# rbrito/deprecated-lame-mirror

Measured on AMD Instinct MI355X. Metric: encoded audio seconds/sec (x real-time) at 44.1kHz stereo CBR128, higher is better.
Workload: dtype f32

## Files before the change

### deprecated-lame-mirror_amd/csrc/lh_dev_common.h

```cpp
#ifndef LH_DEV_COMMON_H
#define LH_DEV_COMMON_H

#include <stdint.h>
#include "lamehip_types.h"
#include "lh_device.h"
#include "lh_wave.h"
#include "lh_dev_math.h"

#define LH_NT 128
#ifdef LH_LSF
#define LH_NGR 1
#define LH_IS_LSF 1
#define LH_RATE8K(c) ((c).rate8k)
#else
#define LH_NGR 2
#define LH_IS_LSF 0
#define LH_RATE8K(c) 0
#endif
#define LH_BLOCK LH_NT
#define LH_SQRT2 1.41421356237309504880

#ifdef LH_EMU
#define LH_SYNC_WG() do { __syncthreads(); } while (0)
#define LH_SYNC_WG_LDS() do { __syncthreads(); } while (0)
// ... 284 lines not shown

struct LhVbrSave {
    uint8_t sfwork[LH_SFBMAX + 1];
    uint8_t sfmin[LH_SFBMAX + 1];
    int     mingain_l, mingain_s[3];
    int     global_gain, mnc, max_bits, use_bits;
    int     ath_over, nonzero, pad[2];
    int     table_select[3], region0_count, region1_count, pad2[3];
};

#if !(defined(LH_PROF) && !defined(LH_EMU))
#define LH_VBR_OLD 1
#endif

struct LhVbrOldSave {
    LhQR    R;
    LhGrR   g;
    uint8_t sf[LH_SFBMAX + 1];
    float   xmin[LH_SFBMAX + 1];
    int     used_bits, fin_bits;
    int     ath_over, pad;
};

struct LhQuantLds {
    LhChanLds ch[2];
};
static_assert(__builtin_offsetof(LhTables, pow43) % 128 == 0 && __builtin_offsetof(LhTables, vqthr) % 128 == 0
              && __builtin_offsetof(LhTables, vq3) % 128 == 0,
              "the gathered tables start on cache lines (hipMalloc aligns the struct itself)");
static_assert(sizeof(LhChanLds) % 16 == 0, "both channels' float2/float4 accesses need 16-byte alignment");
static_assert(__builtin_offsetof(LhPsyLds, mid.small) >= __builtin_offsetof(LhChanLds, ix[1]) + sizeof(((LhChanLds *) 0)->ix[1])
              && __builtin_offsetof(LhPsyLds, mid.lng) + sizeof(LhMidLong) <= sizeof(LhChanLds) + __builtin_offsetof(LhChanLds, ix[1])
              && __builtin_offsetof(LhPsyLds, mid.small) % 16 == 0,
              "the staged mid record lies between the two channels' second images (log table / VBR step tables)");

#define LH_VBR_IPOW20 ((float *) lh_lds.u.quant.ch[0].ix[1])
#define LH_VBR_POW20  ((float *) lh_lds.u.quant.ch[1].ix[1])

#define LH_LOGT_SPLIT 288
#define LH_LOGT_LDS(m) (((const float *) lh_lds.u.quant.ch[0].ix[1]) \
                        [(m) + ((m) >= LH_LOGT_SPLIT ? (int) ((sizeof(LhChanLds) - 4 * LH_LOGT_SPLIT) / 4) : 0)])
#define LH_LOGT_LDS_W(m) (((float *) lh_lds.u.quant.ch[0].ix[1]) \
                          [(m) + ((m) >= LH_LOGT_SPLIT ? (int) ((sizeof(LhChanLds) - 4 * LH_LOGT_SPLIT) / 4) : 0)])
static_assert(sizeof(((LhChanLds *) 0)->ix[1]) == 4 * LH_LOGT_SPLIT && 2 * LH_LOGT_SPLIT >= 513, "log table over the second images");

struct LhCtxShared {
// ... 68 lines not shown
    int8_t  ns_attacks[4][4];
    int     ns_uselong[4];
    int     uselongblock[2];
    int     next_blocktype[2];
    int     block_type[2][2];
    int     mode_ext, padding, mean_bits, max_bits, frame_bits;
    int     targ_bits[2];
    int     bits_used[2];
    float   pe_use[2][2];
    float   ms_ener_ratio[2];
    int     scfsi[2][4];
    int     gr0_done[2];
#if defined(LH_PROF) && !defined(LH_EMU)
    unsigned prof[2][LH_NPROF];
#endif
    LhCtxShared ctx;
    LhRgSlot rg[2];
    union __attribute__((aligned(16))) {
        float   mf[2][LH_MF_NEEDED];
        struct {
            float   xr[2][2][576];
            LhQTabs qt;
            union {
                LhVbrSave vbr[2][2];
#ifdef LH_VBR_OLD
                LhVbrOldSave old[2][2];
#endif
            };
        };
    };
    union __attribute__((aligned(16))) {
        LhPsyLds psy;
        LhMdctLds mdct;
        LhQuantLds quant;
    } u;
};

static_assert(sizeof(LhLds) <= 40960, "four workgroups per CU need <= 40 KiB of the 160 KiB LDS each");

__shared__ LhLds lh_lds __attribute__((aligned(16)));
#define LH_QT (&lh_lds.qt)
#endif

struct LhCtx {
    const LhConfig *cfg;
    const LhTables *T;
    LhStreamState *st;
// ... 313 lines not shown
```

### deprecated-lame-mirror_amd/csrc/lh_dev_qloop.h

```cpp
#ifndef LH_DEV_QLOOP_H
#define LH_DEV_QLOOP_H

#include "lh_dev_quant.h"


struct LhQS {
    float   xp[10];
    uint32_t pw[5];
    int     bnd[5];
    uint32_t vm[5];
    int     bigq;
    int     bq[5];
    float   lmax;
    int     sfw, sfbest;
    float   rxmin;
    int     wid, sta, win, pre;
    int     pnstep;
    float   pnnoise, pnlog;
    float   dist;
    int     ph;
    int     tselw, tselb;
    float   istepv, thrv;
    int     sbg8;
    int     sfbl;
// ... 61 lines not shown
    return __builtin_amdgcn_ldexpf(v, e);
#endif
}

LH_DEVFN int
lq_quant_line_hbm(const LhTables * T, float istep, float xp)
{
    double  x0 = (double) (istep * xp);
    float   f;
    int     k;
    x0 += LH_MAGIC_FLOAT;
    f = (float) x0;
    k = (int) lh_f32_as_u32(f) - LH_MAGIC_INT;
    f = (float) (x0 + T->adj43asm[k]);
    return (int) lh_f32_as_u32(f) - LH_MAGIC_INT;
}

LH_DEVFN void
lq_load(const LhCtx & c, LhQS & S, LhChanLds & Q, const LhQR & R, const LhGrR & g, int qch)
{
    const LhQTabs *qt = LH_QT;
    int const pm = R.mnc >> 1;
    float   mx = 0.0f;
    LH_WAVE_SYNC();
#pragma unroll
    for (int k = 0; k < 5; k++) {
        int const p = c.lane + 64 * k;
        int const ok = (k < 4 || p < 288);
        int const pc = ok ? p : 287;
        lh_f32x2 const x = ((const lh_f32x2 *) Q.xrpow)[pc];
        int const b = Q.sfb_of_line[2 * pc];
        S.xp[2 * k] = ok ? x.x : 0.0f;
        S.xp[2 * k + 1] = ok ? x.y : 0.0f;
        S.bnd[k] = ok ? b : 63;
        S.vm[k] = (ok && p <= pm) ? 0xffffffffu : 0u;
        S.bq[k] = (ok && p <= pm) ? b : 31;
        S.pw[k] = 0u;
        mx = S.xp[2 * k] > mx ? S.xp[2 * k] : mx;
        mx = S.xp[2 * k + 1] > mx ? S.xp[2 * k + 1] : mx;
    }
    S.lmax = mx;
    {
        int const s = c.lane <= LH_SFBMAX ? c.lane : LH_SFBMAX;
        S.sfw = 0;
        S.sfbest = 0;
        S.rxmin = 1.f / Q.l3_xmin[s];
        S.wid = Q.width[s];
        S.sta = Q.start[s];
        S.win = Q.window[s];
        S.pre = (c.lane < LH_SBMAX_L) ? (int) qt->pretab[c.lane < 22 ? c.lane : 0] : 0;
        S.pnstep = 0;
        S.pnnoise = 0;
        S.pnlog = 0;
        S.dist = 0;
        S.ph = Q.pseudohalf[s];
    }
    S.zk = 0;
    S.bigq = 0;
    S.nzend = 0;
    S.tselw = 0;
    S.tselb = S.tselw;
    S.m0 = lh_uni_f(c.T->pow20[210 + LH_QMAX2]);
    S.m1 = lh_uni_f(c.T->pow20[211 + LH_QMAX2]);
    S.m2 = lh_uni_f(c.T->pow20[212 + LH_QMAX2]);
    S.m3 = lh_uni_f(c.T->pow20[213 + LH_QMAX2]);
    S.istepv = c.T->ipow20[210 + (c.lane & 15)];
    S.thrv = (LH_IXMAX) / S.istepv;
    if (c.lane >= 32)
        S.istepv = (1.0f - 0.4054f) / S.istepv;
    S.sbg8 = 0;
    S.sfbl = (c.lane < LH_SBMAX_L + 1) ? (int) qt->sfb_l[c.lane < LH_SBMAX_L + 1 ? c.lane : 0] : 576;
    LH_WAVE_SYNC();
    {
        const uint32_t *hg = c.T->hgrid;
        uint32_t w[11];
#pragma unroll
        for (int j = 0; j < 11; j++)
            w[j] = hg[c.lane + 64 * j];
#pragma unroll
        for (int j = 0; j < 4; j++) {
            Q.hl3_big[0][c.lane + 64 * j] = w[j];
            Q.hl3_big[1][c.lane + 64 * j] = w[4 + j];
        }
#pragma unroll
        for (int j = 0; j < 3; j++)
            Q.hl3_small[c.lane + 64 * j] = w[8 + j];
    }
    if (S.pad) {
        uint32_t const w8 = (c.lane < LH_SBPSY_L) ? (uint32_t) ((S.wid + 7) & ~7) : 0u;
        uint32_t const upto = lh_wave_scan_u32(w8);
        S.sqb = (int) (upto - w8);
#pragma unroll
        for (int k = 0; k < 5; k++) {
            int const b = S.bnd[k] & 63;
            int const at = (int) lh_shfl_u32((uint32_t) S.sqb, b) + 2 * (c.lane + 64 * k) - (int) lh_shfl_u32((uint32_t) S.sta, b);
            S.sqi[k] = 4u * (uint32_t) ((S.bnd[k] < LH_SBPSY_L && S.vm[k]) ? at : LQ_SQ_DUMP);
        }
        LH_WAVE_SYNC();
        for (int i = c.lane; i < 576 / 4; i += 64) {
            lh_f32x4 z;
            z.x = z.y = z.z = z.w = 0.0f;
            ((lh_f32x4 *) Q.xrpow)[i] = z;
        }
    }
    LH_WAVE_SYNC();
}

template < int USE_PREV, int NS > LH_DEVFN int
lq_quantize(const LhCtx & c, LhQS & S, const LhQR & R, const LhGrR & g)
// ... 490 lines not shown
                 "v_cmpx_gt_i32_e64 %[tm], %[rem], 24\n\t"
                 LQ_OCT(240, 241, 242, 243, 244, 245, 246, 247)
                 "v_add_u32_e32 %[rem], -32, %[rem]\n\t"
                 "v_add_u32_e32 %[ad], 0x80, %[ad]\n\t"
                 "v_cmpx_gt_i32_e64 %[tm], %[rem], 0\n\t"
                 "s_cbranch_execnz .Llq_sum_loop_%=\n\t"
                 ".Llq_sum_done_%=:\n\t"
                 "s_mov_b64 exec, %[sv]\n\t"
                 "s_waitcnt lgkmcnt(0)"
                 : [ns] "+v"(noise), [rem] "+v"(rem), [ad] "+v"(ad), [sv] "=&s"(sv_), [tm] "=&s"(tm_)
                 :
                 : "memory", "v192", "v193", "v194", "v195", "v196", "v197", "v198", "v199", "v208", "v209", "v210", "v211",
                   "v212", "v213", "v214", "v215", "v224", "v225", "v226", "v227", "v228", "v229", "v230", "v231",
                   "v240", "v241", "v242", "v243", "v244", "v245", "v246", "v247");
#undef LQ_OCT
#else
    for (int i = 0; i < n; i++)
        noise += sq[base + i];
#endif
    return noise;
}

template < int NS > LH_DEVFN void
lq_zero_band_noise(const LhCtx & c, LhQS & S, const LhQR & R, LhChanLds & Q, const float *xr)
{
    float  *sq = Q.xrpow;
    int const s = c.lane;
    int const mine = (s < R.psymax);
    int     l = 0, j = 0, maxw;
    if (mine) {
        l = S.wid >> 1;
        j = S.sta;
        if ((j + S.wid) > R.mnc) {
            int const usefullsize = R.mnc - j + 1;
            l = (usefullsize > 0) ? (usefullsize >> 1) : 0;
        }
    }
    LH_WAVE_SYNC();
#pragma unroll
    for (int k = 0; k < NS; k++) {
        int const p = c.lane + 64 * k;
        lh_f32x2 const ax = ((const lh_f32x2 *) xr)[(k < 4 || c.lane < 32) ? c.lane + 64 * k : 287];
        float const t0 = lh_fabsf(ax.x), t1 = lh_fabsf(ax.y);
        lh_f32x2 v;
        v.x = t0 * t0;
        v.y = t1 * t1;
        if (S.pad)
            *(lh_f32x2 *) ((char *) sq + S.sqi[k]) = v;
        else if (k < 4 || p < 288)
            ((lh_f32x2 *) sq)[p] = v;
    }
    LH_WAVE_ORDER();
    maxw = (int) lh_wave_max_u32(mine ? (unsigned) (2 * l) : 0u);
    S.zk = S.pad ? lq_band_sums_pad(sq, S.sqb, mine ? 2 * l : 0, maxw) : lq_band_sums(sq, 2 * l, (j < 576) ? (j >> 1) : 0, maxw, mine);
    LH_WAVE_SYNC();
}

struct LhNoiseTmp {
    int     pnstep;
    float   pnnoise, pnlog, dist;
    LhNoiseRes res;
};

LH_DEVFN float
lq_pow20_of_step(const LhQS & S, int st)
{
    int const d = st - 210, q = d >> 2, r = d & 3;
    float const m0 = lh_uni_f(S.m0), m1 = lh_uni_f(S.m1), m2 = lh_uni_f(S.m2), m3 = lh_uni_f(S.m3);
    float const m = (r & 2) ? ((r & 1) ? m3 : m2) : ((r & 1) ? m1 : m0);
    return lq_ldexp(m, q);
}

template < int NS > LH_DEVFN void
lq_noise_squares(const LhCtx & c, const LhQS & S, const LhGrR & g, LhChanLds & Q, const float *xr)
{
    const LhTables *T = c.T;
    const LhQTabs *qt = LH_QT;
// ... 558 lines not shown

template < int NS, int SPEC = 0, int SHORT = 0 > LH_DEVFN void
lq_stage_body(int qch, int gr, int targ_bits)
{
    LhCtx   c = lh_ctx_load();
    LhQR    R = lh_uniform(lh_lds.rg[qch].R);
    LhGrR   g = lh_uniform(lh_lds.rg[qch].g);
    if (SPEC) {
        lh_pin_usual(c, SPEC);
        if (SHORT) {
            c.subblock_gain = 1;
            lh_pin_usual_short(R);
        }
        else
            lh_pin_usual(R);
    }
    LhChanLds & Q = lh_lds.u.quant.ch[qch];
    LhQS    S;
    S.pad = (SPEC != 0 && !SHORT);
    R.s_mnc = lh_uni_i((int) Q.sfb_of_line[R.mnc]);
#if defined(LH_TRACE) && !defined(LH_EMU)
    lh_tr_begin(S.tr);
#endif
    lq_load(c, S, Q, R, g, qch);
    LQ_T(S, 51);
    lq_zero_band_noise < NS > (c, S, R, Q, lh_lds.xr[qch][lh_uni_i(gr)]);
    LQ_T(S, 52);
    (void) lq_outer_loop < NS > (c, S, Q, R, g, lh_lds.xr[qch][lh_uni_i(gr)], qch, lh_uni_i(targ_bits));
    LQ_T(S, 53);
    LQ_T(S, 63);
    lh_rg_put(c, R, g);
#if defined(LH_TRACE) && !defined(LH_EMU)
    lh_tr_flush(S.tr, c.wave);
#endif
}

#ifdef LH_VBR_OLD
template < int NS, int SPEC = 0 > LH_DEVFN void
lq_vbrold_body(int qch, int gr, int min_bits, int max_bits, int cont)
{
    LhCtx   c = lh_ctx_load();
    LhQR    R = lh_uniform(lh_lds.rg[qch].R);
    LhGrR   g = lh_uniform(lh_lds.rg[qch].g);
    if (SPEC) {
        c.ns = 1;
        c.ns_amp = 1;
        c.full_outer_loop = 0;
        c.sfb21_extra = (SPEC == 2);
        c.rate8k = 0;
// ... 3 lines not shown
        R.psy_lmax = (SPEC == 2) ? LH_SBMAX_L : LH_SBPSY_L;
        R.psymax = R.psy_lmax;
        R.sfbmax = LH_SBPSY_L;
        R.sfbdivide = 11;
        if ((R.substep_shaping & 2) != 0)
            __builtin_unreachable();
    }
    LhChanLds & Q = lh_lds.u.quant.ch[qch];
    const float *xr = lh_lds.xr[qch][lh_uni_i(gr)];
    LhQS    S;
    LhQOld  K;
    LhGrR   gbst = g;
    float   xpbst[10], lmaxbst = 0.0f;
    uint32_t pwbst[5] = { 0u, 0u, 0u, 0u, 0u };
    int     sfbst = 0, tselbst = 0;
    int const band = c.lane <= LH_SFBMAX ? c.lane : LH_SFBMAX;
    int     found = 0, dbits, this_bits;
    min_bits = lh_uni_i(min_bits);
    max_bits = lh_uni_i(max_bits);
    int const top = max_bits;
    R.s_mnc = lh_uni_i((int) Q.sfb_of_line[R.mnc]);
    S.pad = 0;
    lq_load(c, S, Q, R, g, qch);
    lq_zero_band_noise < NS > (c, S, R, Q, xr);
    if (lh_uni_i(cont)) {
        S.sfw = Q.sf[0][band];
        S.sfbest = S.sfw;
        S.sbg8 = 8 * lh_sbg(g, S.win);
        S.tselw = (c.lane == 0) ? g.table_select[0] : (c.lane == 1) ? g.table_select[1] : g.table_select[2];
        S.tselb = S.tselw;
    }
#pragma unroll
    for (int k = 0; k < 10; k++)
        xpbst[k] = 0.0f;
    this_bits = (max_bits + min_bits) / 2;
    do {
        int const sfb21 = c.sfb21_extra && !(this_bits > top - 42);
        int const over = lq_outer_loop < NS, 1 > (c, S, Q, R, g, xr, qch, this_bits, sfb21, &K);
        if (over <= 0) {
            found = 1;
            gbst = g;
            sfbst = S.sfbest;
            tselbst = S.tselb;
            lmaxbst = S.lmax;
#pragma unroll
            for (int k = 0; k < 10; k++)
                xpbst[k] = S.xp[k];
// ... 160 lines not shown
```

### deprecated-lame-mirror_amd/csrc/lh_dev_quant.h

```cpp
#ifndef LH_DEV_QUANT_H
#define LH_DEV_QUANT_H

#include "lh_dev_common.h"

#define LH_MAGIC_FLOAT (65536*(128))
#define LH_MAGIC_INT 0x4b000000

LH_DEVCONST int lh_slen1_n[16] = { 1, 1, 1, 1, 8, 2, 2, 2, 4, 4, 4, 8, 8, 8, 16, 16 };
LH_DEVCONST int lh_slen2_n[16] = { 1, 2, 4, 8, 1, 2, 4, 8, 2, 4, 8, 2, 4, 8, 4, 8 };
LH_DEVCONST int lh_slen1_tab[16] = { 0, 0, 0, 0, 3, 1, 1, 1, 2, 2, 2, 3, 3, 3, 4, 4 };
LH_DEVCONST int lh_slen2_tab[16] = { 0, 1, 2, 3, 0, 1, 2, 3, 1, 2, 3, 1, 2, 3, 2, 3 };
LH_DEVCONST int lh_scfsi_band[5] = { 0, 6, 11, 16, 21 };
LH_DEVCONST int lh_scale_short[16] = { 0, 18, 36, 54, 54, 36, 54, 72, 54, 72, 90, 72, 90, 108, 108, 126 };
LH_DEVCONST int lh_scale_long[16] = { 0, 10, 20, 30, 33, 21, 31, 41, 32, 42, 52, 43, 53, 63, 64, 74 };
LH_DEVCONST int lh_huf_tbl_noESC[15] = { 1, 2, 5, 7, 7, 10, 10, 13, 13, 13, 13, 13, 13, 13, 13 };

LH_DEVFN int
lh_ht_off(int t)
{
    switch (t) {
    case 1: return 0;
    case 2: return 4;
    case 3: return 13;
    case 5: return 22;
// ... 516 lines not shown
    float   lx, lv = 0.0f;
    if (logt_lds) {
        LH_FAST_LOG2_VIA(LH_LOGT_LDS, x, lx);
        if (v > 1E-20f)
            LH_FAST_LOG2_VIA(LH_LOGT_LDS, v, lv);
    }
    else {
        lx = lh_fast_log2(T->log_table, x);
        if (v > 1E-20f)
            lv = lh_fast_log2(T->log_table, v);
    }
    float   u = (float) (lx * (LH_LOG2_OVER_LOG10 * (10.0f)));
    float   w = 0.0f;
    u -= athFloor;
    if (v > 1E-20f)
        w = (float) (1.f + lv * (LH_LOG2_OVER_LOG10 * (10.0f / o)));
    if (w < 0)
        w = 0.f;
    u *= w;
    u += athFloor + o - p;
    return lh_powf(10.f, 0.1f * u);
}

LH_DEVFN void
lh_calc_xmin_body(const LhCtx & c, LhChanLds & Q, LhQR & R, const float *xr, const float *ren, const float *rthm)
{
    const LhConfig *cfg = c.cfg;
    const LhTables *T = c.T;
    const LhQTabs *qt = LH_QT;
    int const s = c.lane;
    float const adj = lh_lds.ss.ath_adjust_factor;
    int const logt_lds = lh_uni_i(!(cfg->vbr == 1 || cfg->vbr == 4));
    int     over = 0;
    if (s < R.psymax) {
        int const is_long = (s < R.psy_lmax);
        int const sfb = is_long ? s : (R.sfb_smin + (s - R.psy_lmax) / 3);
        int const b = is_long ? 0 : (s - R.psy_lmax) % 3;
        float   en0 = 0.0f, xmin, ath, rh1, rh2, rh3, fact, e, t;
        int const width = Q.width[s];
        int     j = Q.start[s];
        if (is_long) {
            ath = lh_ath_adjust(T, adj, T->ath_l[sfb], T->ath_floor, cfg->ATHfixpoint, logt_lds);
            fact = T->longfact[sfb];
            e = ren[sfb];
            t = rthm[sfb];
        }
        else {
            ath = lh_ath_adjust(T, adj, T->ath_s[sfb], T->ath_floor, cfg->ATHfixpoint, logt_lds);
            fact = T->shortfact[sfb];
            e = ren[22 + sfb * 3 + b];
            t = rthm[22 + sfb * 3 + b];
        }
        ath *= fact;
        rh1 = ath / width;
        rh2 = (float) 2.2204460492503131e-16;
        {
            const lh_f32x2 *xp = (const lh_f32x2 *) (xr + j);
            int const np = width >> 1;
            int     p = 0;
            lh_f32x2 n0 = xp[0], n1 = xp[1], n2 = xp[2], n3 = xp[3];
            for (; p + 4 <= np; p += 4) {
                lh_f32x2 const a0 = n0, a1 = n1, a2 = n2, a3 = n3;
                n0 = xp[p + 4];
                n1 = xp[p + 5];
                n2 = xp[p + 6];
                n3 = xp[p + 7];
#ifndef LH_EMU
                {
                    float   t_;
#define LH_XM_TERM(X) "v_mul_f32 %[t], %[" #X "], %[" #X "]\n\tv_add_f32 %[en], %[en], %[t]\n\tv_min_f32 %[t], %[t], %[rh1]\n\tv_add_f32 %[rh2], %[rh2], %[t]\n\t"
                    asm volatile(LH_XM_TERM(a0) LH_XM_TERM(a1) LH_XM_TERM(a2) LH_XM_TERM(a3)
                                 LH_XM_TERM(a4) LH_XM_TERM(a5) LH_XM_TERM(a6) LH_XM_TERM(a7)
                                 : [en] "+v"(en0), [rh2] "+v"(rh2), [t] "=&v"(t_)
                                 : [rh1] "v"(rh1), [a0] "v"(a0.x), [a1] "v"(a0.y), [a2] "v"(a1.x), [a3] "v"(a1.y),
                                   [a4] "v"(a2.x), [a5] "v"(a2.y), [a6] "v"(a3.x), [a7] "v"(a3.y));
#undef LH_XM_TERM
// ... 13 lines not shown
                float   x2 = a0.x * a0.x;
                en0 += x2;
                rh2 += (x2 < rh1) ? x2 : rh1;
                x2 = a0.y * a0.y;
                en0 += x2;
                rh2 += (x2 < rh1) ? x2 : rh1;
            }
        }
        if (en0 < ath)
            rh3 = en0;
        else if (rh2 < ath)
            rh3 = ath;
        else
            rh3 = rh2;
        xmin = rh3;
        if (e > 1e-12f) {
            float   x = en0 * t / e;
            x *= fact;
            if (xmin < x)
                xmin = x;
        }
        xmin = (float) ((xmin > 2.2204460492503131e-16) ? xmin : 2.2204460492503131e-16);
        Q.l3_xmin[s] = xmin;
        Q.sfb_mode[s] = (en0 > xmin + 1e-14f) ? 1 : 0;
        over = (en0 > ath);
    }
    R.ath_over = (lh_ballot(over) != 0);
    {
        unsigned top = 0;
        int     max_nonzero;
        for (int k = c.lane; k < 576; k += 64)
            if (k > 0 && lh_fabsf(xr[k]) > 1e-12f)
                top = (unsigned) k;
        top = lh_wave_max_u32(top);
        max_nonzero = (int) top;
        if (R.block_type != LH_SHORT_TYPE)
            max_nonzero |= 1;
        else {
            max_nonzero /= 6;
            max_nonzero *= 6;
            max_nonzero += 5;
        }
        if (c.sfb21_extra == 0 && cfg->samplerate < 44000) {
            int     limit;
            if (R.block_type != LH_SHORT_TYPE)
                limit = qt->sfb_l[LH_RATE8K(c) ? 17 : 21] - 1;
// ... 5 lines not shown
        R.mnc = max_nonzero;
    }
    LH_WAVE_SYNC();
    if (cfg->use_temporal_masking && s < R.psymax && s >= R.psy_lmax && ((s - R.psy_lmax) % 3) == 0) {
        float   x0 = Q.l3_xmin[s], x1 = Q.l3_xmin[s + 1], x2 = Q.l3_xmin[s + 2];
        if (x0 > x1)
            x1 += (x0 - x1) * T->decay;
        if (x1 > x2)
            x2 += (x1 - x2) * T->decay;
        Q.l3_xmin[s + 1] = x1;
        Q.l3_xmin[s + 2] = x2;
    }
    LH_WAVE_SYNC();
}

LH_STAGEFN void
lh_calc_xmin(int qch, int gr, int rch)
{
    LhCtx const c = lh_ctx_load();
    LhQR    R = lh_uniform(lh_lds.rg[qch].R);
    {
        int const slot = (lh_uni_i(lh_lds.psy_slot) + gr) % 3;
        lh_calc_xmin_body(c, lh_lds.u.quant.ch[qch], R, lh_lds.xr[qch][gr], lh_lds.psy_en[slot][rch],
                          lh_lds.psy_thm[slot][rch]);
    }
    if (c.lane == 0)
        lh_lds.rg[qch].R = R;
    LH_WAVE_SYNC();
}

LH_STAGEFN void
lh_calc_xmin_n(int qch, int gr, int rch)
{
    LhCtx   c = lh_ctx_load();
    LhQR    R = lh_uniform(lh_lds.rg[qch].R);
    lh_pin_usual(c, 0);
    lh_pin_usual(R);
    {
        int const slot = (lh_uni_i(lh_lds.psy_slot) + gr) % 3;
        lh_calc_xmin_body(c, lh_lds.u.quant.ch[qch], R, lh_lds.xr[qch][gr], lh_lds.psy_en[slot][rch],
                          lh_lds.psy_thm[slot][rch]);
    }
    if (c.lane == 0)
        lh_lds.rg[qch].R = R;
    LH_WAVE_SYNC();
}

LH_DEVFN void
lh_init_outer_loop_body(const LhCtx & c, LhChanLds & Q, LhQR & R, LhGrR & g, float *xr, int block_type, int substep,
                        int reorder = 1)
{
    const LhTables *T = c.T;
    const LhQTabs *qt = LH_QT;
    int const sfb21 = c.sfb21_extra;
    g.part2_3_length = 0;
    g.big_values = 0;
    g.count1 = 0;
    g.global_gain = 210;
    g.scalefac_compress = 0;
    g.table_select[0] = g.table_select[1] = g.table_select[2] = 0;
    g.subblock_gain[0] = g.subblock_gain[1] = g.subblock_gain[2] = g.subblock_gain[3] = 0;
    g.region0_count = g.region1_count = 0;
    g.preflag = 0;
    g.scalefac_scale = 0;
    g.count1table_select = 0;
    g.part2_length = 0;
    g.count1bits = 0;
    g.xrpow_max = 0;
    R.block_type = block_type;
    R.sfb_lmax = LH_RATE8K(c) ? 17 : LH_SBPSY_L;
    R.sfb_smin = LH_RATE8K(c) ? 9 : LH_SBPSY_S;
    R.psy_lmax = LH_RATE8K(c) ? 17 : (sfb21 ? LH_SBMAX_L : LH_SBPSY_L);
    R.psymax = R.psy_lmax;
// ... 24 lines not shown
            Q.width[s] = 0;
            Q.window[s] = 3;
            Q.start[s] = 576;
        }
        else if (block_type == LH_SHORT_TYPE) {
            int const sfb = s / 3, win = s - 3 * sfb;
            int const wd = T->sfb_s[sfb + 1] - T->sfb_s[sfb];
            Q.width[s] = wd;
            Q.window[s] = win;
            Q.start[s] = 3 * T->sfb_s[sfb] + win * wd;
        }
        else if (s < LH_SBMAX_L) {
            Q.width[s] = qt->sfb_l[s + 1] - qt->sfb_l[s];
            Q.window[s] = 3;
            Q.start[s] = qt->sfb_l[s];
        }
        else {
            Q.width[s] = 0;
            Q.window[s] = 3;
            Q.start[s] = 576;
        }
    }
    LH_WAVE_SYNC();
    {
        const uint32_t *src = (const uint32_t *) ((block_type == LH_SHORT_TYPE) ? T->sfb_line_s : T->sfb_line_l);
        uint32_t *dst = (uint32_t *) Q.sfb_of_line;
        uint32_t const a = src[c.lane], b = src[c.lane + 64], d = src[(c.lane < 16) ? c.lane + 128 : 0];
        dst[c.lane] = a;
        dst[c.lane + 64] = b;
        if (c.lane < 16)
            dst[c.lane + 128] = d;
    }
    if (block_type == LH_SHORT_TYPE && reorder) {
        float  *tmp = Q.save_xrpow;
        for (int i = c.lane; i < 576; i += 64)
            tmp[i] = xr[i];
        LH_WAVE_SYNC();
        for (int d = c.lane; d < 576; d += 64) {
            int     sfb = 0;
            for (int k = 1; k < LH_SBMAX_S; k++)
                if (3 * T->sfb_s[k] <= d)
                    sfb = k;
            {
                int const wd = T->sfb_s[sfb + 1] - T->sfb_s[sfb];
                int const r = d - 3 * T->sfb_s[sfb];
                int const win = r / wd, l = T->sfb_s[sfb] + (r - win * wd);
                xr[d] = tmp[3 * l + win];
// ... 1 lines not shown
        }
    }
    LH_WAVE_SYNC();
}

LH_STAGEFN void
lh_init_outer_loop(int qch, int gr, int block_type, int substep, int reorder = 1)
{
    LhCtx const c = lh_ctx_load();
    LhQR    R;
    LhGrR   g;
    lh_init_outer_loop_body(c, lh_lds.u.quant.ch[qch], R, g, lh_lds.xr[qch][gr], lh_uni_i(block_type),
                            lh_uni_i(substep), lh_uni_i(reorder));
    lh_rg_put(c, R, g);
}

LH_STAGEFN void
lh_init_outer_loop_n(int qch, int gr, int substep)
{
    LhCtx   c = lh_ctx_load();
    LhQR    R;
    LhGrR   g;
    lh_pin_usual(c, 0);
    lh_init_outer_loop_body(c, lh_lds.u.quant.ch[qch], R, g, lh_lds.xr[qch][gr], LH_NORM_TYPE, lh_uni_i(substep), 0);
    lh_rg_put(c, R, g);
}

LH_DEVFN void
lh_zero_tail(const LhCtx & c, LhChanLds & Q, const LhQR & R)
{
    for (int i = c.lane; i < 576; i += 64)
        if (i > R.mnc)
            Q.ix[0][i] = 0;
    LH_WAVE_SYNC();
}

LH_DEVFN int
lh_init_xrpow(const LhCtx & c, LhChanLds & Q, const LhQR & R, LhGrR & g, const float *xr)
{
    unsigned mxabs = 0, mxpow = 0;
    int     nonzero;
    for (int i = c.lane; i < 576; i += 64) {
        float const tmp = (i <= R.mnc) ? lh_fabsf(xr[i]) : 0.0f;
        float const xp = (float) sqrt((double) tmp * sqrt((double) tmp));
        unsigned const ub = lh_f32_as_u32(tmp), up = lh_f32_as_u32(xp);
        Q.xrpow[i] = xp;
        mxabs = ub > mxabs ? ub : mxabs;
// ... 695 lines not shown
```

### deprecated-lame-mirror_amd/csrc/lh_dev_vbr.h

```cpp
#ifndef LH_DEV_VBR_H
#define LH_DEV_VBR_H

#include "lh_dev_quant.h"

LH_DEVFN int
lh_imax(int a, int b)
{
    return a > b ? a : b;
}

LH_DEVFN int
lh_imin(int a, int b)
{
    return a < b ? a : b;
}

LH_DEVFN int
lh_wave_max0(int v)
{
    return (int) lh_wave_max_u32((unsigned) (v > 0 ? v : 0));
}

LH_DEVFN int
lh_wave_min_i32(int v)
// ... 634 lines not shown
        c.rate8k = 0;
        pass = 0;
    }
    LhChanLds & Q = L.u.quant.ch[qch];
    LhVbrSave & sv = L.vbr[gr][qch];
    float  *xr = L.xr[qch][gr];
    int const s = c.lane;
    int const sc = s < LH_SFBMAX ? s : LH_SFBMAX;
    LhQR    R;
    LhGrR   g;
    int     live, nonzero, sfw = 0, sfm = 0, mingain_l = 0, mingain_s[3] = { 0, 0, 0 };
    gr = lh_uni_i(gr);
    pass = lh_uni_i(pass);
    gate = lh_uni_i(gate);
    target = lh_uni_i(target);

    LH_PT(t_q);
    LH_PT(t_a);
    lh_init_outer_loop_body(c, Q, R, g, xr, USUAL ? LH_NORM_TYPE : lh_uni_i(L.block_type[gr][qch]), lh_uni_i(substep), pass == 0);
    LH_PA(15, t_a);
    if (pass == 0) {
        {
            int const slot = (lh_uni_i(L.psy_slot) + gr) % 3;
            lh_calc_xmin_body(c, Q, R, xr, L.psy_en[slot][rch], L.psy_thm[slot][rch]);
            LH_WAVE_SYNC();
            LH_DBG_XMIN(c, gr, qch, rch, Q, R.psymax);
        }
    }
    else {
        R.mnc = lh_uni_i(sv.mnc);
        g.table_select[0] = lh_uni_i(sv.table_select[0]);
        g.table_select[1] = lh_uni_i(sv.table_select[1]);
        g.table_select[2] = lh_uni_i(sv.table_select[2]);
        g.region0_count = lh_uni_i(sv.region0_count);
        g.region1_count = lh_uni_i(sv.region1_count);
    }
    LH_PA(16, t_a);
    nonzero = lh_init_xrpow(c, Q, R, g, xr);
    if (pass == 0 && !nonzero)
        LH_ROUTE(c, LH_ROUTE_ZERO(R.block_type));
    if (pass == 0 && s == 0) {
        sv.mnc = R.mnc;
        sv.ath_over = R.ath_over;
        sv.nonzero = nonzero;
    }
    live = nonzero && gate > 0;
    LH_PA(4, t_a);
// ... 411 lines not shown
```

### deprecated-lame-mirror_amd/csrc/lh_kernels.hip

```cpp
#include <stdint.h>
#include <math.h>

#ifdef LH_EMU
#include "hipemu.h"
#define LH_CONST static const
#else
#include <hip/hip_runtime.h>
#define LH_CONST __device__ static const
#endif

#ifdef LH_EMU
#include <string.h>
#if defined(LH_LSF) || defined(LH_SPLIT)
extern "C" { extern int lh_emu_poison_lds; }
#else
extern "C" { int lh_emu_poison_lds = 0; }
#endif
#endif
#include "lh_static_tables.h"
#include "lh_dev_common.h"
#include "lh_dev_psy.h"
#include "lh_dev_mdct.h"
#include "lh_dev_quant.h"
#include "lh_dev_qloop.h"

LH_DEVFN void
lh_adjust_ATH(const LhTables * T, const float loud[2][2], float *factor, float *limit)
{
    float const was = *factor, floor_was = *limit;
    float   level, now, floor_now;
    if (T->ath_use_adjust == 0) {
        *factor = 1.0;
        return;
    }
    {
        float const first = loud[0][0] + loud[0][1], second = loud[1][0] + loud[1][1];
        level = (first > second) ? first : second;
        level = (float) (level * 0.5);
        level *= T->aa_sensitivity_p;
// ... 64 lines not shown
}

LH_DEVFN void
lh_stage_loop_tables(const LhCtx & c)
{
    const LhTables *T = c.T;
    lh_load_qtabs(c, lh_lds.qt);
    if (c.cfg->vbr == 1 || c.cfg->vbr == 4) {
        for (int i = c.tid; i < 256; i += LH_NT) {
            LH_VBR_IPOW20[i] = T->ipow20[i];
            LH_VBR_POW20[i] = T->pow20[i + LH_QMAX2];
        }
    }
    else {
        for (int i = c.tid; i < 513; i += LH_NT)
            LH_LOGT_LDS_W(i) = T->log_table[i];
    }
}

LH_DEVFN void
lh_store_granule(const LhCtx & c, const LhChanLds & Q, const LhQR & R, const LhGrR & g,
                 const float *xr, LhGranule * o)
{
    const int16_t *ix = Q.ix[0];
    for (int i = c.lane; i < 576; i += 64) {
        int     v = ix[i];
        if (v != 0 && xr[i] < 0.0f)
            v = -v;
        o->l3_enc[i] = (int16_t) v;
    }
    if (c.lane < LH_SFBMAX)
        o->scalefac[c.lane] = (int8_t) Q.sf[0][c.lane];
    if (c.lane == 0) {
        o->pad0 = 0;
        o->part2_3_length = (int16_t) g.part2_3_length;
        o->part2_length = (int16_t) g.part2_length;
        o->big_values = (int16_t) g.big_values;
        o->count1 = (int16_t) g.count1;
        o->global_gain = (int16_t) g.global_gain;
        o->scalefac_compress = (int16_t) g.scalefac_compress;
        o->block_type = (int8_t) R.block_type;
        o->mixed_block_flag = 0;
#pragma unroll
        for (int i = 0; i < 3; i++) {
            o->table_select[i] = (int8_t) g.table_select[i];
            o->subblock_gain[i] = (int8_t) g.subblock_gain[i];
        }
        o->region0_count = (int8_t) g.region0_count;
        o->region1_count = (int8_t) g.region1_count;
        o->preflag = (int8_t) g.preflag;
        o->scalefac_scale = (int8_t) g.scalefac_scale;
        o->count1table_select = (int8_t) g.count1table_select;
// ... 27 lines not shown
#define LH_DBG_XMIN(c, gr, ch, rch, Q, psymax) lh_dbg_xmin(c, gr, ch, rch, Q, psymax)
#define LH_DBG_XR(c, gr, ch, xr) lh_dbg_xr(c, gr, ch, xr)
#else
#define LH_DBG_XMIN(c, gr, ch, rch, Q, psymax) do { } while (0)
#define LH_DBG_XR(c, gr, ch, xr) do { } while (0)
#endif

#include "lh_dev_emit.h"
#include "lh_dev_vbr.h"
#ifdef LH_VBR_OLD
#include "lh_dev_vbrold.h"
#endif

LH_DEVFN int
lh_prepare_granule(const LhCtx & c, int ch, int gr, int msoff, int substep)
{
    LhLds & L = lh_lds;
    LhChanLds & Q = L.u.quant.ch[ch];
    LhQR    R;
    LhGrR   g;
    int     nonzero;
    int const usual = lh_uni_i(lh_granule_is_usual(c, L.block_type[gr][ch], substep));
    LH_ROUTE(c, usual ? LH_RT_PREP_n : LH_RT_PREP_gen);
    if (usual)
        lh_init_outer_loop_n(ch, gr, substep);
    else
        lh_init_outer_loop(ch, gr, L.block_type[gr][ch], substep);
    R = lh_uniform(L.rg[ch].R);
    g = lh_uniform(L.rg[ch].g);
    nonzero = lh_init_xrpow(c, Q, R, g, L.xr[ch][gr]);
    if (nonzero) {
        lh_rg_put(c, R, g);
        if (usual)
            lh_calc_xmin_n(ch, gr, msoff + ch);
        else
            lh_calc_xmin(ch, gr, msoff + ch);
        R = lh_uniform(L.rg[ch].R);
        LH_DBG_XMIN(c, gr, ch, msoff + ch, Q, R.psymax);
        lh_zero_tail(c, Q, R);
    }
    lh_rg_put(c, R, g);
    return lh_uni_i(nonzero);
}


#if !defined(LH_EMU)
static __device__ int lh_prio_tab[8 * 8 * 2 * 16 * 4 * 2];
LH_DEVFN int
lh_prio_index()
{
    unsigned v, x;
    asm volatile("s_getreg_b32 %0, hwreg(HW_REG_HW_ID)" : "=s"(v));
    asm volatile("s_getreg_b32 %0, hwreg(HW_REG_XCC_ID)" : "=s"(x));
// ... 118 lines not shown
        for (int gr = 0; gr < ngr; gr++) {
            float   r = L.tot_ener[gr][2] + L.tot_ener[gr][3];
            if (r > 0)
                r = L.tot_ener[gr][3] / r;
            ms_ener_ratio[gr] = lh_uni_f(r);
        }
    }

    {
        float   factor = lh_lds.ss.ath_adjust_factor, limit = lh_lds.ss.ath_adjust_limit;
        float   loud[2][2];
        loud[0][0] = L.loudness_sq[0][0];
        loud[1][0] = L.loudness_sq[ngr - 1][0];
        loud[0][1] = (cfg->channels == 2) ? L.loudness_sq[0][1] : loud[0][0];
        loud[1][1] = (cfg->channels == 2) ? L.loudness_sq[ngr - 1][1] : loud[1][0];
        lh_adjust_ATH(T, loud, &factor, &limit);
        LH_SYNC_WG();
        if (tid == 0) {
            lh_lds.ss.ath_adjust_factor = factor;
            lh_lds.ss.ath_adjust_limit = limit;
        }
    }
    LH_SYNC_WG();

    LH_PA(25, t_frame);
    LH_PT(t_mdct);
#ifndef LH_SPLIT
#pragma unroll
    for (int k = 0; k < 9; k++)
        L.u.mdct.sb[w][0][lane + 64 * k] = carry.sb[k];
    lh_polyphase(w);
    LH_SYNC_WG();
    lh_mdct_granules(w);
#pragma unroll
    for (int k = 0; k < 9; k++)
        carry.sb[k] = L.u.mdct.sb[w][ngr][lane + 64 * k];
    LH_SYNC_WG();
#endif
    LH_PA(2, t_mdct);
#ifndef LH_SPLIT
    lh_stage_loop_tables(c);
    LH_SYNC_WG();
#endif

    int     mode_ext = LH_MPG_MD_LR_LR;
    if (cfg->force_ms)
        mode_ext = LH_MPG_MD_MS_LR;
    else if (cfg->mode == LH_MODE_JOINT_STEREO) {
        float   sum_pe_MS = 0, sum_pe_LR = 0;
        for (int gr = 0; gr < ngr; gr++)
            for (int ch = 0; ch < 2; ch++) {
                sum_pe_MS += L.pe[gr][2 + ch];
                sum_pe_LR += L.pe[gr][ch];
            }
        if (sum_pe_MS <= 1.00 * sum_pe_LR) {
            if (L.block_type[0][0] == L.block_type[0][1] && L.block_type[ngr - 1][0] == L.block_type[ngr - 1][1])
                mode_ext = LH_MPG_MD_MS_LR;
        }
    }
    mode_ext = lh_uni_i(mode_ext);
    int const msoff = (mode_ext == LH_MPG_MD_MS_LR) ? 2 : 0;

    float   pe_use[2][2];
    {
        float   buf[19], f;
// ... 388 lines not shown
    c.d.pcm_r = lh_uni_ll(c.d.pcm_r);
    c.d.pcm_base = lh_uni_ll(c.d.pcm_base);
    c.d.nsamples = lh_uni_ll(c.d.nsamples);
    c.d.out_index = lh_uni_ll(c.d.out_index);
    c.d.frame_begin = lh_uni_i(c.d.frame_begin);
    c.d.frame_end = lh_uni_i(c.d.frame_end);
    c.d.bytes_base = lh_uni_ll(c.d.bytes_base);
    c.d.bytes_cap = lh_uni_ll(c.d.bytes_cap);
    c.d.flush = lh_uni_i(c.d.flush);
    c.d.mid_rel = lh_uni_i(c.d.mid_rel);
    c.tid = (int) threadIdx.x;
    c.lane = c.tid & 63;
    c.wave = lh_uni_i(c.tid >> 6);
    lh_ctx_hot(c);
    if (c.tid == 0) {
        L.gr0_done[0] = L.gr0_done[1] = 0;
        L.ctx.cfg = c.cfg;
        L.ctx.T = c.T;
        L.ctx.st = c.st;
        L.ctx.pcm = c.pcm;
        L.ctx.pcmf = c.pcmf;
        L.ctx.bytes = bytes;
        L.ctx.d = c.d;
    }
    LhWaveCarry carry;
    carry.prio_rel = 0;
    carry.prio_late = 0;
    LhStreamState *st = c.st;
    for (int p = 0; p < 2; p++) {
        carry.nb.n1[p] = st->nb_l1[c.wave + 2 * p][c.lane];
        carry.nb.n2[p] = st->nb_l2[c.wave + 2 * p][c.lane];
    }
#ifndef LH_SPLIT
#pragma unroll
    for (int k = 0; k < 9; k++)
        carry.sb[k] = st->sb_prev[c.wave][c.lane + 64 * k];
#endif
    for (int t = c.tid; t < 4 * LH_XMIN_N; t += LH_NT) {
        int const chn = t / LH_XMIN_N, i = t - chn * LH_XMIN_N;
        L.psy_en[0][chn][i] = st->en[chn][i];
        L.psy_thm[0][chn][i] = st->thm[chn][i];
    }
    if (c.tid < LH_SS_WORDS_A)
        ((uint32_t *) &L.ss)[c.tid] = ((const uint32_t *) &st->loudness_sq_save[0])[c.tid];
    else if (c.tid < LH_SS_WORDS_A + LH_SS_WORDS_B)
        ((uint32_t *) &L.ss)[c.tid] = ((const uint32_t *) &st->pefirbuf[0])[c.tid - LH_SS_WORDS_A];
// ... 279 lines not shown
```

Before: 84110.

## Cache per-band ATH values in LDS and reuse band energies for zero-band noise

Adds an LDS cache of per-band ATH and scale factors, keyed on the ATH adjust factor, so calc_xmin reads them instead of recomputing powf-based adjustments every granule. It also stores band energies from calc_xmin and reuses them in zero-band noise when whole bands are in range, skipping the band-sum pass. Global table loads in lq_load are hoisted ahead of the LDS work, the sfb_of_line copy is moved to overlap with init_xrpow, and granule stores are widened to 32-bit pairs. The cost is extra LDS space in a union and cache invalidation logic, with emulator checks added to verify the cached values match.

```diff
diff --git a/deprecated-lame-mirror_amd/csrc/lh_dev_common.h b/deprecated-lame-mirror_amd/csrc/lh_dev_common.h
--- a/deprecated-lame-mirror_amd/csrc/lh_dev_common.h
+++ b/deprecated-lame-mirror_amd/csrc/lh_dev_common.h
@@ -330,6 +330,17 @@
     int     ath_over, pad;
 };
 
+#define LH_ATHC_N (LH_SBMAX_L + LH_SBMAX_S)
+struct LhAthCache {
+    float   ath[LH_ATHC_N];
+    float   fact[LH_ATHC_N];
+    uint32_t key;
+    int     valid;
+};
+#ifdef LH_EMU
+extern "C" { extern long long lh_emu_granule_check[10]; }
+#endif
+
 struct LhQuantLds {
     LhChanLds ch[2];
 };
@@ -444,7 +455,10 @@
             float   xr[2][2][576];
             LhQTabs qt;
             union {
-                LhVbrSave vbr[2][2];
+                struct {
+                    LhVbrSave vbr[2][2];
+                    LhAthCache athc;
+                };
 #ifdef LH_VBR_OLD
                 LhVbrOldSave old[2][2];
 #endif
diff --git a/deprecated-lame-mirror_amd/csrc/lh_dev_qloop.h b/deprecated-lame-mirror_amd/csrc/lh_dev_qloop.h
--- a/deprecated-lame-mirror_amd/csrc/lh_dev_qloop.h
+++ b/deprecated-lame-mirror_amd/csrc/lh_dev_qloop.h
@@ -107,6 +107,16 @@
     const LhQTabs *qt = LH_QT;
     int const pm = R.mnc >> 1;
     float   mx = 0.0f;
+    uint32_t hw[11];
+    {
+        const uint32_t *hg = c.T->hgrid;
+#pragma unroll
+        for (int j = 0; j < 11; j++)
+            hw[j] = hg[c.lane + 64 * j];
+    }
+    float const pw0 = c.T->pow20[210 + LH_QMAX2], pw1 = c.T->pow20[211 + LH_QMAX2], pw2 = c.T->pow20[212 + LH_QMAX2],
+        pw3 = c.T->pow20[213 + LH_QMAX2];
+    float const ipw = c.T->ipow20[210 + (c.lane & 15)];
     LH_WAVE_SYNC();
 #pragma unroll
     for (int k = 0; k < 5; k++) {
@@ -145,11 +155,11 @@
     S.nzend = 0;
     S.tselw = 0;
     S.tselb = S.tselw;
-    S.m0 = lh_uni_f(c.T->pow20[210 + LH_QMAX2]);
-    S.m1 = lh_uni_f(c.T->pow20[211 + LH_QMAX2]);
-    S.m2 = lh_uni_f(c.T->pow20[212 + LH_QMAX2]);
-    S.m3 = lh_uni_f(c.T->pow20[213 + LH_QMAX2]);
-    S.istepv = c.T->ipow20[210 + (c.lane & 15)];
+    S.m0 = lh_uni_f(pw0);
+    S.m1 = lh_uni_f(pw1);
+    S.m2 = lh_uni_f(pw2);
+    S.m3 = lh_uni_f(pw3);
+    S.istepv = ipw;
     S.thrv = (LH_IXMAX) / S.istepv;
     if (c.lane >= 32)
         S.istepv = (1.0f - 0.4054f) / S.istepv;
@@ -157,19 +167,14 @@
     S.sfbl = (c.lane < LH_SBMAX_L + 1) ? (int) qt->sfb_l[c.lane < LH_SBMAX_L + 1 ? c.lane : 0] : 576;
     LH_WAVE_SYNC();
     {
-        const uint32_t *hg = c.T->hgrid;
-        uint32_t w[11];
-#pragma unroll
-        for (int j = 0; j < 11; j++)
-            w[j] = hg[c.lane + 64 * j];
 #pragma unroll
         for (int j = 0; j < 4; j++) {
-            Q.hl3_big[0][c.lane + 64 * j] = w[j];
-            Q.hl3_big[1][c.lane + 64 * j] = w[4 + j];
+            Q.hl3_big[0][c.lane + 64 * j] = hw[j];
+            Q.hl3_big[1][c.lane + 64 * j] = hw[4 + j];
         }
 #pragma unroll
         for (int j = 0; j < 3; j++)
-            Q.hl3_small[c.lane + 64 * j] = w[8 + j];
+            Q.hl3_small[c.lane + 64 * j] = hw[8 + j];
     }
     if (S.pad) {
         uint32_t const w8 = (c.lane < LH_SBPSY_L) ? (uint32_t) ((S.wid + 7) & ~7) : 0u;
@@ -706,18 +711,44 @@
 }
 
 template < int NS > LH_DEVFN void
-lq_zero_band_noise(const LhCtx & c, LhQS & S, const LhQR & R, LhChanLds & Q, const float *xr)
+lq_zero_band_noise(const LhCtx & c, LhQS & S, const LhQR & R, LhChanLds & Q, const float *xr, int parked)
 {
     float  *sq = Q.xrpow;
     int const s = c.lane;
     int const mine = (s < R.psymax);
     int     l = 0, j = 0, maxw;
+    float   en0 = 0.0f;
     if (mine) {
         l = S.wid >> 1;
         j = S.sta;
         if ((j + S.wid) > R.mnc) {
             int const usefullsize = R.mnc - j + 1;
             l = (usefullsize > 0) ? (usefullsize >> 1) : 0;
+        }
+    }
+#ifdef LH_EMU
+    int const l_all = l;
+#define LQ_ZK_CHECK() do { if (parked && mine) { \
+            float ref_ = 0.0f; \
+            for (int i_ = 0; i_ < 2 * l_all; i_++) { float const t_ = lh_fabsf(xr[j + i_]); ref_ += t_ * t_; } \
+            lh_emu_granule_check[0]++; \
+            lh_emu_granule_check[1] += (lh_f32_as_u32(ref_) != lh_f32_as_u32(S.zk)); } \
+        if (parked) { uint64_t const cut_ = lh_ballot(mine && l_all > 0 && l_all < (S.wid >> 1)); \
+            if (s == 0) { lh_emu_granule_check[cut_ ? 2 : 7]++; \
+                lh_emu_granule_check[R.block_type == LH_SHORT_TYPE ? 9 : 8] |= (long long) cut_; } } } while (0)
+#else
+#define LQ_ZK_CHECK() do { } while (0)
+#endif
+    if (parked) {
+        int const whole = mine && l == (S.wid >> 1);
+        if (whole)
+            en0 = Q.sfb_f[s];
+        l = whole ? 0 : l;
+        if (lh_ballot(l > 0) == 0) {
+            S.zk = en0;
+            LQ_ZK_CHECK();
+            LH_WAVE_SYNC();
+            return;
         }
     }
     LH_WAVE_SYNC();
@@ -737,6 +768,10 @@
     LH_WAVE_ORDER();
     maxw = (int) lh_wave_max_u32(mine ? (unsigned) (2 * l) : 0u);
     S.zk = S.pad ? lq_band_sums_pad(sq, S.sqb, mine ? 2 * l : 0, maxw) : lq_band_sums(sq, 2 * l, (j < 576) ? (j >> 1) : 0, maxw, mine);
+    if (parked && l == 0)
+        S.zk = en0;
+    LQ_ZK_CHECK();
+#undef LQ_ZK_CHECK
     LH_WAVE_SYNC();
 }
 
@@ -1341,9 +1376,12 @@
 #if defined(LH_TRACE) && !defined(LH_EMU)
     lh_tr_begin(S.tr);
 #endif
+    LH_PT(t_se);
     lq_load(c, S, Q, R, g, qch);
+    LH_PA(38, t_se);
     LQ_T(S, 51);
-    lq_zero_band_noise < NS > (c, S, R, Q, lh_lds.xr[qch][lh_uni_i(gr)]);
+    lq_zero_band_noise < NS > (c, S, R, Q, lh_lds.xr[qch][lh_uni_i(gr)], 1);
+    LH_PA(39, t_se);
     LQ_T(S, 52);
     (void) lq_outer_loop < NS > (c, S, Q, R, g, lh_lds.xr[qch][lh_uni_i(gr)], qch, lh_uni_i(targ_bits));
     LQ_T(S, 53);
@@ -1393,7 +1431,7 @@
     R.s_mnc = lh_uni_i((int) Q.sfb_of_line[R.mnc]);
     S.pad = 0;
     lq_load(c, S, Q, R, g, qch);
-    lq_zero_band_noise < NS > (c, S, R, Q, xr);
+    lq_zero_band_noise < NS > (c, S, R, Q, xr, 0);
     if (lh_uni_i(cont)) {
         S.sfw = Q.sf[0][band];
         S.sfbest = S.sfw;
diff --git a/deprecated-lame-mirror_amd/csrc/lh_dev_quant.h b/deprecated-lame-mirror_amd/csrc/lh_dev_quant.h
--- a/deprecated-lame-mirror_amd/csrc/lh_dev_quant.h
+++ b/deprecated-lame-mirror_amd/csrc/lh_dev_quant.h
@@ -562,15 +562,61 @@
     return lh_powf(10.f, 0.1f * u);
 }
 
+LH_DEVFN float
+lh_ath_band(const LhCtx & c, float adj, int at, float *fact)
+{
+    const LhTables *T = c.T;
+    int const logt_lds = lh_uni_i(!(c.cfg->vbr == 1 || c.cfg->vbr == 4));
+    int const is_long = (at < LH_SBMAX_L);
+    float const a = is_long ? T->ath_l[at] : T->ath_s[at - LH_SBMAX_L];
+    float const f = is_long ? T->longfact[at] : T->shortfact[at - LH_SBMAX_L];
+    float   ath = lh_ath_adjust(T, adj, a, T->ath_floor, c.cfg->ATHfixpoint, logt_lds);
+    ath *= f;
+    *fact = f;
+    return ath;
+}
+
+LH_DEVFN int
+lh_ath_cached(const LhCtx & c)
+{
+    return lh_uni_i(c.cfg->vbr != 2);
+}
+
 LH_DEVFN void
-lh_calc_xmin_body(const LhCtx & c, LhChanLds & Q, LhQR & R, const float *xr, const float *ren, const float *rthm)
+lh_ath_cache_update(const LhCtx & c, int always)
+{
+    LhAthCache & A = lh_lds.athc;
+    if (c.wave != 0 || !lh_ath_cached(c))
+        return;
+    float const adj = lh_lds.ss.ath_adjust_factor;
+    int const stale = lh_uni_i(always || !A.valid || A.key != lh_f32_as_u32(adj));
+    LH_WAVE_SYNC();
+#ifdef LH_EMU
+    if (c.lane == 0)
+        lh_emu_granule_check[stale ? 5 : 6]++;
+#endif
+    if (!stale)
+        return;
+    if (c.lane < LH_ATHC_N) {
+        float   fact;
+        float const ath = lh_ath_band(c, adj, c.lane, &fact);
+        A.ath[c.lane] = ath;
+        A.fact[c.lane] = fact;
+    }
+    if (c.lane == 0) {
+        A.key = lh_f32_as_u32(adj);
+        A.valid = 1;
+    }
+    LH_WAVE_SYNC();
+}
+
+LH_DEVFN void
+lh_calc_xmin_body(const LhCtx & c, LhChanLds & Q, LhQR & R, const float *xr, const float *ren, const float *rthm, int cached)
 {
     const LhConfig *cfg = c.cfg;
     const LhTables *T = c.T;
     const LhQTabs *qt = LH_QT;
     int const s = c.lane;
-    float const adj = lh_lds.ss.ath_adjust_factor;
-    int const logt_lds = lh_uni_i(!(cfg->vbr == 1 || cfg->vbr == 4));
     int     over = 0;
     if (s < R.psymax) {
         int const is_long = (s < R.psy_lmax);
@@ -579,19 +625,29 @@
         float   en0 = 0.0f, xmin, ath, rh1, rh2, rh3, fact, e, t;
         int const width = Q.width[s];
         int     j = Q.start[s];
+        int const at = is_long ? sfb : LH_SBMAX_L + sfb;
+        if (cached) {
+            ath = lh_lds.athc.ath[at];
+            fact = lh_lds.athc.fact[at];
+#ifdef LH_EMU
+            {
+                float   f_;
+                float const a_ = lh_ath_band(c, lh_lds.ss.ath_adjust_factor, at, &f_);
+                lh_emu_granule_check[3]++;
+                lh_emu_granule_check[4] += (lh_f32_as_u32(a_) != lh_f32_as_u32(ath) || lh_f32_as_u32(f_) != lh_f32_as_u32(fact));
+            }
+#endif
+        }
+        else
+            ath = lh_ath_band(c, lh_lds.ss.ath_adjust_factor, at, &fact);
         if (is_long) {
-            ath = lh_ath_adjust(T, adj, T->ath_l[sfb], T->ath_floor, cfg->ATHfixpoint, logt_lds);
-            fact = T->longfact[sfb];
             e = ren[sfb];
             t = rthm[sfb];
         }
         else {
-            ath = lh_ath_adjust(T, adj, T->ath_s[sfb], T->ath_floor, cfg->ATHfixpoint, logt_lds);
-            fact = T->shortfact[sfb];
             e = ren[22 + sfb * 3 + b];
             t = rthm[22 + sfb * 3 + b];
         }
-        ath *= fact;
         rh1 = ath / width;
         rh2 = (float) 2.2204460492503131e-16;
         {
@@ -651,6 +707,7 @@
         }
         xmin = (float) ((xmin > 2.2204460492503131e-16) ? xmin : 2.2204460492503131e-16);
         Q.l3_xmin[s] = xmin;
+        Q.sfb_f[s] = en0;
         Q.sfb_mode[s] = (en0 > xmin + 1e-14f) ? 1 : 0;
         over = (en0 > ath);
     }
@@ -702,7 +759,7 @@
     {
         int const slot = (lh_uni_i(lh_lds.psy_slot) + gr) % 3;
         lh_calc_xmin_body(c, lh_lds.u.quant.ch[qch], R, lh_lds.xr[qch][gr], lh_lds.psy_en[slot][rch],
-                          lh_lds.psy_thm[slot][rch]);
+                          lh_lds.psy_thm[slot][rch], lh_ath_cached(c));
     }
     if (c.lane == 0)
         lh_lds.rg[qch].R = R;
@@ -719,7 +776,7 @@
     {
         int const slot = (lh_uni_i(lh_lds.psy_slot) + gr) % 3;
         lh_calc_xmin_body(c, lh_lds.u.quant.ch[qch], R, lh_lds.xr[qch][gr], lh_lds.psy_en[slot][rch],
-                          lh_lds.psy_thm[slot][rch]);
+                          lh_lds.psy_thm[slot][rch], 1);
     }
     if (c.lane == 0)
         lh_lds.rg[qch].R = R;
@@ -728,7 +785,7 @@
 
 LH_DEVFN void
 lh_init_outer_loop_body(const LhCtx & c, LhChanLds & Q, LhQR & R, LhGrR & g, float *xr, int block_type, int substep,
-                        int reorder = 1)
+                        int reorder = 1, int lines = 1)
 {
     const LhTables *T = c.T;
     const LhQTabs *qt = LH_QT;
@@ -799,7 +856,7 @@
         }
     }
     LH_WAVE_SYNC();
-    {
+    if (lines) {
         const uint32_t *src = (const uint32_t *) ((block_type == LH_SHORT_TYPE) ? T->sfb_line_s : T->sfb_line_l);
         uint32_t *dst = (uint32_t *) Q.sfb_of_line;
         uint32_t const a = src[c.lane], b = src[c.lane + 64], d = src[(c.lane < 16) ? c.lane + 128 : 0];
@@ -847,7 +904,7 @@
     LhQR    R;
     LhGrR   g;
     lh_pin_usual(c, 0);
-    lh_init_outer_loop_body(c, lh_lds.u.quant.ch[qch], R, g, lh_lds.xr[qch][gr], LH_NORM_TYPE, lh_uni_i(substep), 0);
+    lh_init_outer_loop_body(c, lh_lds.u.quant.ch[qch], R, g, lh_lds.xr[qch][gr], LH_NORM_TYPE, lh_uni_i(substep), 0, 0);
     lh_rg_put(c, R, g);
 }
 
diff --git a/deprecated-lame-mirror_amd/csrc/lh_dev_vbr.h b/deprecated-lame-mirror_amd/csrc/lh_dev_vbr.h
--- a/deprecated-lame-mirror_amd/csrc/lh_dev_vbr.h
+++ b/deprecated-lame-mirror_amd/csrc/lh_dev_vbr.h
@@ -680,7 +680,7 @@
     if (pass == 0) {
         {
             int const slot = (lh_uni_i(L.psy_slot) + gr) % 3;
-            lh_calc_xmin_body(c, Q, R, xr, L.psy_en[slot][rch], L.psy_thm[slot][rch]);
+            lh_calc_xmin_body(c, Q, R, xr, L.psy_en[slot][rch], L.psy_thm[slot][rch], 1);
             LH_WAVE_SYNC();
             LH_DBG_XMIN(c, gr, qch, rch, Q, R.psymax);
         }
diff --git a/deprecated-lame-mirror_amd/csrc/lh_kernels.hip b/deprecated-lame-mirror_amd/csrc/lh_kernels.hip
--- a/deprecated-lame-mirror_amd/csrc/lh_kernels.hip
+++ b/deprecated-lame-mirror_amd/csrc/lh_kernels.hip
@@ -15,6 +15,7 @@
 extern "C" { extern int lh_emu_poison_lds; }
 #else
 extern "C" { int lh_emu_poison_lds = 0; }
+extern "C" { long long lh_emu_granule_check[10] = { 0, 0, 0, 0, 0, 0, 0, 0, 0, 0 }; }
 #endif
 #endif
 #include "lh_static_tables.h"
@@ -125,12 +126,22 @@
 lh_store_granule(const LhCtx & c, const LhChanLds & Q, const LhQR & R, const LhGrR & g,
                  const float *xr, LhGranule * o)
 {
-    const int16_t *ix = Q.ix[0];
-    for (int i = c.lane; i < 576; i += 64) {
-        int     v = ix[i];
-        if (v != 0 && xr[i] < 0.0f)
-            v = -v;
-        o->l3_enc[i] = (int16_t) v;
+    const uint32_t *ix2 = (const uint32_t *) Q.ix[0];
+    const lh_f32x2 *xr2 = (const lh_f32x2 *) xr;
+    uint32_t *enc2 = (uint32_t *) o->l3_enc;
+#pragma unroll
+    for (int k = 0; k < 5; k++) {
+        int const p = c.lane + 64 * k;
+        int const pc = (k < 4 || p < 288) ? p : 287;
+        uint32_t const w = ix2[pc];
+        lh_f32x2 const x = xr2[pc];
+        int     v0 = (int) (int16_t) (w & 0xffffu), v1 = (int) (int16_t) (w >> 16);
+        if (v0 != 0 && x.x < 0.0f)
+            v0 = -v0;
+        if (v1 != 0 && x.y < 0.0f)
+            v1 = -v1;
+        if (k < 4 || p < 288)
+            enc2[p] = ((uint32_t) v0 & 0xffffu) | ((uint32_t) v1 << 16);
     }
     if (c.lane < LH_SFBMAX)
         o->scalefac[c.lane] = (int8_t) Q.sf[0][c.lane];
@@ -204,13 +215,31 @@
     int     nonzero;
     int const usual = lh_uni_i(lh_granule_is_usual(c, L.block_type[gr][ch], substep));
     LH_ROUTE(c, usual ? LH_RT_PREP_n : LH_RT_PREP_gen);
+    LH_PT(t_pg);
     if (usual)
         lh_init_outer_loop_n(ch, gr, substep);
     else
         lh_init_outer_loop(ch, gr, L.block_type[gr][ch], substep);
     R = lh_uniform(L.rg[ch].R);
     g = lh_uniform(L.rg[ch].g);
+    LH_PA(28, t_pg);
+    uint32_t ln0 = 0u, ln1 = 0u, ln2 = 0u;
+    if (usual) {
+        const uint32_t *src = (const uint32_t *) c.T->sfb_line_l;
+        ln0 = src[c.lane];
+        ln1 = src[c.lane + 64];
+        ln2 = src[(c.lane < 16) ? c.lane + 128 : 0];
+    }
     nonzero = lh_init_xrpow(c, Q, R, g, L.xr[ch][gr]);
+    if (usual) {
+        uint32_t *dst = (uint32_t *) Q.sfb_of_line;
+        dst[c.lane] = ln0;
+        dst[c.lane + 64] = ln1;
+        if (c.lane < 16)
+            dst[c.lane + 128] = ln2;
+        LH_WAVE_SYNC();
+    }
+    LH_PA(37, t_pg);
     if (nonzero) {
         lh_rg_put(c, R, g);
         if (usual)
@@ -375,6 +404,9 @@
         }
     }
     LH_SYNC_WG();
+#ifdef LH_SPLIT
+    lh_ath_cache_update(c, 0);
+#endif
 
     LH_PA(25, t_frame);
     LH_PT(t_mdct);
@@ -394,6 +426,7 @@
 #ifndef LH_SPLIT
     lh_stage_loop_tables(c);
     LH_SYNC_WG();
+    lh_ath_cache_update(c, 1);
 #endif
 
     int     mode_ext = LH_MPG_MD_LR_LR;
@@ -828,6 +861,8 @@
         L.ctx.pcmf = c.pcmf;
         L.ctx.bytes = bytes;
         L.ctx.d = c.d;
+        if (lh_ath_cached(c))
+            L.athc.valid = 0;
     }
     LhWaveCarry carry;
     carry.prio_rel = 0;
```

Result: no change. 84630 (median of 6 runs) (+0.6%).
